# Samleo8/RadarSLAMPy

Measured on AMD Instinct MI355X. Metric: radar scan-pairs/sec (400x3768 polar), higher is better.
Workload: dtype u8/f32/f64

## Files before the change

### radarslampy_amd/csrc/engine.hip

```cpp
#include "roam_internal.h"
#include "retrack.h"
#include "kabsch_body.inc"
#include <algorithm>
#include <new>

#define KS ROAM_MAX_FEATURES
#define CART_CENTER 1012.0
#define M_PER_PX 0.0864
#define N_RETRACK 60
#define ROT_THR 0.2
#define TRANS_THR_SQ 4.0
#define ERR_THR 10.0f
#define TWO_PI 6.283185307179586476925286766559

#define RES_RING 8
enum { ST_PEAKS = 0, ST_WARP, ST_PYR, ST_KLT, ST_GRAPH, ST_CLIQUE, ST_KABSCH, ST_LM, ST_GLUE, ST_RETRACK, ST_COUNT };
static const char *kStageNames[ST_COUNT] = {"ingest_peaks", "warp_quantise", "pyramid", "klt", "consistency_graph",
                                            "max_clique", "kabsch", "mds_lm", "glue", "retrack"};

struct Engine {
    roam_engine_cfg cfg;
    int B = 0, W = 0, stage_cap = 0;
    PyrDesc pd;
    size_t rec_bytes = 0;
// ... 532 lines not shown
    if (e->scan_host) hipHostFree(e->scan_host);
    if (e->prior_host) hipHostFree(e->prior_host);
    if (e->results_host) hipHostFree(e->results_host);
    for (auto &ev : e->ev_res) if (ev) hipEventDestroy(ev);
    if (e->st_comm) { hipStreamSynchronize(e->st_comm); hipStreamDestroy(e->st_comm); }
    for (auto &ev : e->ev_kfx) if (ev) hipEventDestroy(ev);
    if (e->ev_pool) hipEventDestroy(e->ev_pool);
    for (auto &ev : e->ev_up_ring) if (ev) hipEventDestroy(ev);
    hipStreamSynchronize(ctx->stream2);
    hipStreamSynchronize(ctx->stream4);
    delete e;
    ctx->engine = nullptr;
    return ROAM_OK;
}

static int32_t fused_tables(roam_ctx *ctx, Engine *e)
{
    RtArgs &r = e->rt;
    if (r.fd_mapT) return ROAM_OK;
    const size_t npx = (size_t)e->W * e->W, R = (size_t)r.slots;
    uint32_t *mapT = nullptr, *boxtab = nullptr, *darktab = nullptr;
    bool ok = dalloc(ctx, e, &mapT, npx) && dalloc(ctx, e, &boxtab, retrack_fused_boxtab_words(e->W)) && dalloc(ctx, e, &darktab, retrack_darktab_words(e->W));
    ok = ok && dalloc(ctx, e, &r.fd_halo, R * 2 * (size_t)r.fd_halo_words) && dalloc(ctx, e, &r.fd_cc, R * 2048);
    if (!ok) return ROAM_E_HIP;
    HIP_TRY(ctx, launch_retrack_fused_tables(ctx->stream, e->warp_map, e->W, e->cfg.clip, mapT, boxtab, darktab));
    HIP_TRY(ctx, hipStreamSynchronize(ctx->stream));
    r.fd_boxtab = boxtab; r.fd_darktab = darktab;
    r.fd_mapT = mapT;
    return ROAM_OK;
}

int32_t roam_engine_create(roam_ctx *ctx, const roam_engine_cfg *cfg)
{
    if (!ctx) return ROAM_E_ARG;
    HIP_TRY(ctx, hipSetDevice(ctx->device));
    ARG_CHECK(ctx, cfg && cfg->lanes >= 1 && cfg->rows >= 1 && cfg->rows <= 1020 && cfg->clip >= 32 && cfg->clip <= 4094 && (cfg->clip / 2) % 2 == 0 &&
                       (int64_t)cfg->rows * cfg->stride < (1ll << 30) &&
                       cfg->payload_off >= 0 && cfg->stride >= cfg->payload_off + cfg->clip && cfg->pool_scans >= 1 &&
                       cfg->peaks_cap >= 1);
    roam_engine_destroy(ctx);
    Engine *e = new (std::nothrow) Engine();
    if (!e) return ROAM_E_HIP;
    ctx->engine = e;
    e->cfg = *cfg;
    if (!(e->cfg.keyframe_trans_m > 0.0)) e->cfg.keyframe_trans_m = 2.0;
    if (!(e->cfg.keyframe_rot_rad > 0.0)) e->cfg.keyframe_rot_rad = ROT_THR;
    const int B = e->B = cfg->lanes;
    e->lane_k.assign(B, 0);
    e->last_scan.assign(B, -1);
    e->prev_scan.assign(B, -1);
    e->lane_seen.assign(B, 0);
    e->slot_writes.assign((size_t)cfg->pool_scans, 0);
    e->W = 2 * (cfg->clip / 2);
    e->stage_cap = (cfg->clip + 1) / 2;
    pyr_desc_init(&e->pd, e->W, e->W);
    e->rec_bytes = (size_t)cfg->rows * cfg->stride;
    const int nw = KS / 64;
    bool ok = true;
    ok = ok && dalloc(ctx, e, &e->pool, e->rec_bytes * cfg->pool_scans + 64);
    ok = ok && dalloc(ctx, e, &e->pyr[0], (size_t)e->pd.lane_stride * B);
    ok = ok && dalloc(ctx, e, &e->pyr[1], (size_t)e->pd.lane_stride * B);
    ok = ok && dalloc(ctx, e, &e->pyr[2], (size_t)e->pd.lane_stride * B);
    ok = ok && dalloc(ctx, e, &e->pyr[3], (size_t)e->pd.lane_stride * B);
    ok = ok && dalloc(ctx, e, &e->pyr_dark, pyr_dark_words(e->W));
    ok = ok && dalloc(ctx, e, &e->warp_map, (size_t)e->W * e->W);
    ok = ok && dalloc(ctx, e, &e->row_stage, (size_t)B * cfg->rows * e->stage_cap);
    ok = ok && dalloc(ctx, e, &e->row_count, (size_t)B * cfg->rows);
    for (int i = 0; i < 3; i++) {
        ok = ok && dalloc(ctx, e, &e->peaks_out[i], (size_t)B * cfg->peaks_cap * 2);
        ok = ok && dalloc(ctx, e, &e->peaks_n[i], (size_t)B);
        ok = ok && dalloc(ctx, e, &e->scan_idx[i], 2 * (size_t)B);
    }
    if (ok && hipHostMalloc(reinterpret_cast<void **>(&e->scan_host), sizeof(int32_t) * 6 * (size_t)B, hipHostMallocDefault) != hipSuccess) {
        ROAM_SET_ERR(ctx, "engine: hipHostMalloc failed"); ok = false;
    }
    e->prior_bytes = ((size_t)B * 25 + 15) & ~(size_t)15;
    if (ok && hipHostMalloc(reinterpret_cast<void **>(&e->prior_host), 4 * e->prior_bytes, hipHostMallocDefault) != hipSuccess) {
        ROAM_SET_ERR(ctx, "engine: hipHostMalloc failed"); ok = false;
    }
    ok = ok && dalloc(ctx, e, &e->prior_dev, 4 * e->prior_bytes);
    ok = ok && dalloc(ctx, e, &e->feat, (size_t)B * KS * 2);
    ok = ok && dalloc(ctx, e, &e->feat_n, (size_t)B);
    ok = ok && dalloc(ctx, e, &e->klt_next, (size_t)B * KS * 2);
    ok = ok && dalloc(ctx, e, &e->klt_err, (size_t)B * KS);
    ok = ok && dalloc(ctx, e, &e->klt_status, (size_t)B * KS);
    ok = ok && dalloc(ctx, e, &e->good_old, (size_t)B * KS * 2);
    ok = ok && dalloc(ctx, e, &e->good_new, (size_t)B * KS * 2);
    ok = ok && dalloc(ctx, e, &e->good_idx, (size_t)B * KS);
    ok = ok && dalloc(ctx, e, &e->good_n, (size_t)B);
    ok = ok && dalloc(ctx, e, &e->adj, (size_t)B * KS * nw);
    ok = ok && dalloc(ctx, e, &e->cq_stack, (size_t)B * (KS + 2) * 2 * nw);
    ok = ok && dalloc(ctx, e, &e->cq_order, (size_t)B);
    ok = ok && dalloc(ctx, e, &e->cq_mask, (size_t)B * KS);
    ok = ok && dalloc(ctx, e, &e->cq_n, (size_t)B);
    ok = ok && dalloc(ctx, e, &e->cq_flags, (size_t)B);
    ok = ok && dalloc(ctx, e, &e->kab_src, (size_t)B * KS * 2);
    ok = ok && dalloc(ctx, e, &e->kab_tgt, (size_t)B * KS * 2);
    ok = ok && dalloc(ctx, e, &e->kab_out, (size_t)B * 6);
    ok = ok && dalloc(ctx, e, &e->in_n, (size_t)B);
    ok = ok && dalloc(ctx, e, &e->kf_pose, (size_t)B * 3);
    ok = ok && dalloc(ctx, e, &e->kf_vel, (size_t)B * 3) && dalloc(ctx, e, &e->kf_scan, (size_t)B) && dalloc(ctx, e, &e->kf_fresh, (size_t)B) &&
         dalloc(ctx, e, &e->kf_live, (size_t)B) && dalloc(ctx, e, &e->map_n, (size_t)B);
    ok = ok && dalloc(ctx, e, &e->kf_und, (size_t)B * KS * 2);
    ok = ok && dalloc(ctx, e, &e->kf_und_tmp, (size_t)B * KS * 2);
    ok = ok && dalloc(ctx, e, &e->pose, (size_t)B * 3);
    ok = ok && dalloc(ctx, e, &e->vel, (size_t)B * 3);
    ok = ok && dalloc(ctx, e, &e->T_wj0, (size_t)B * 9);
    ok = ok && dalloc(ctx, e, &e->T_init, (size_t)B * 9);
    ok = ok && dalloc(ctx, e, &e->p_w, (size_t)B * KS * 2);
    ok = ok && dalloc(ctx, e, &e->p_jt, (size_t)B * KS * 2);
    ok = ok && dalloc(ctx, e, &e->lm_work, (size_t)B * ((size_t)(2 * KS + 3) * 9 + KS));
    ok = ok && dalloc(ctx, e, &e->lm_out, (size_t)B * 6);
    ok = ok && dalloc(ctx, e, &e->lm_nfev, (size_t)B);
    ok = ok && dalloc(ctx, e, &e->lm_big, (size_t)2 * (1 + B));
    ok = ok && dalloc(ctx, e, &e->lm_info, (size_t)B);
    ok = ok && dalloc(ctx, e, &e->results, (size_t)B * RES_RING);
    if (ok && hipHostMalloc(reinterpret_cast<void **>(&e->results_host), sizeof(roam_lane_result) * (size_t)B * RES_RING, hipHostMallocDefault) != hipSuccess) {
        ROAM_SET_ERR(ctx, "engine: hipHostMalloc failed"); ok = false;
    }
    { const char *se = getenv("ROAM_STAGE_EVENTS"); e->stage_ev = !(se && se[0] == '0'); e->stage_ev_forced = se && (se[0] == '0' || se[0] == '1'); }
    e->rt_on = cfg->retrack_on_device != 0;
    if (ok && e->rt_on) {
        RtArgs &r = e->rt;
        memset(&r, 0, sizeof(r));
        const double step = (10.0 - 0.01) / 2.0;
        r.sigma1 = 1.0 * step + 0.01; r.sigma2 = 10.0; r.threshold = 0.0005;
        r.size1 = (int)(3 * r.sigma1); r.size2 = (int)(3 * r.sigma2);
        r.W = e->W; r.rows = cfg->rows; r.cols = cfg->clip; r.stride = cfg->stride; r.payload_off = cfg->payload_off;
        r.rec_bytes = (int64_t)e->rec_bytes;
        const int R = r.slots = std::max(1, std::min(B, cfg->retrack_slots > 0 ? cfg->retrack_slots : 2048));
        const size_t npx = (size_t)e->W * e->W;
        if (e->W > 2048) { ROAM_SET_ERR(ctx, "engine: device retrack needs a Cartesian image of at most 2048 x 2048"); roam_engine_destroy(ctx); return ROAM_E_ARG; }
        ok = ok && dalloc(ctx, e, &r.rt_n, 2) && dalloc(ctx, e, &r.rt_lane, (size_t)B) && dalloc(ctx, e, &r.rt_scan, (size_t)B);
        r.SP = (e->W + 15) & ~15;
        ok = ok && dalloc(ctx, e, &r.S, (size_t)r.SP * e->W * R);
        ok = ok && dalloc(ctx, e, const_cast<uint32_t **>(&r.boxtab), retrack_boxtab_words(e->W));
        ok = ok && dalloc(ctx, e, const_cast<uint32_t **>(&r.darktab), retrack_darktab_words(e->W));
        ok = ok && dalloc(ctx, e, const_cast<uint32_t **>(&r.phlist), retrack_phase_words(e->W));
        ok = ok && dalloc(ctx, e, &r.colT, (size_t)std::min(R, RT_TWO_PASS_SLOTS) * ((e->W + 63) / 64) * e->W);
        ok = ok && dalloc(ctx, e, &r.col_done, (size_t)std::min(R, RT_TWO_PASS_SLOTS) * 64);
        {
            const char *fv = getenv("ROAM_FUSED_DETECT");
            r.fused = (fv && fv[0] == '1') ? 1 : 0;
            e->det_side.chunk = getenv("ROAM_DET_SIDE") ? atoi(getenv("ROAM_DET_SIDE")) : ((B >= 2048 && r.slots >= 2048) ? 1024 : 0);
            r.fd_halo_words = (int64_t)retrack_fused_halo_words(e->W);
        }
        const size_t D = (size_t)B;
        ok = ok && dalloc(ctx, e, &r.cand_rc, D * BP_MAX_PTS) && dalloc(ctx, e, &r.cand_val, D * BP_MAX_PTS) && dalloc(ctx, e, &r.cand_n, D);
        ok = ok && dalloc(ctx, e, &r.tasks, D * BP_MAX_TASKS) && dalloc(ctx, e, &r.pairs, D * (BP_MAX_PAIRS + 1));
        ok = ok && dalloc(ctx, e, &r.order, D * (BP_MAX_PAIRS + 1)) && dalloc(ctx, e, &r.ovbits, D * ((BP_MAX_PAIRS + 31) / 32 + 1));
        ok = ok && dalloc(ctx, e, &r.bigtab, D * 2 * 131072);
        ok = ok && dalloc(ctx, e, &r.kp, D * BP_MAX_PTS * 3) && dalloc(ctx, e, &r.kp_n, D) && dalloc(ctx, e, &r.slot_flags, D);
        ok = ok && dalloc(ctx, e, &r.ssc_work, D * 4 * BP_MAX_PTS) && dalloc(ctx, e, &r.sel, D * BP_MAX_PTS) && dalloc(ctx, e, &r.sel_n, D) && dalloc(ctx, e, &r.blob_order_buf, D);
    }
    if (!ok) { roam_engine_destroy(ctx); return ROAM_E_HIP; }
    if (e->rt_on) {
        if (hipError_t er = retrack_init(); er != hipSuccess) {
            ROAM_SET_ERR(ctx, "retrack_init failed: %s", hipGetErrorString(er));
            roam_engine_destroy(ctx);
            return ROAM_E_HIP;
        }
        RtArgs &r = e->rt;
        r.pool = e->pool; r.map = e->warp_map; r.feat = e->feat; r.feat_n = e->feat_n; r.vel = e->vel; r.kf_und = e->kf_und; r.res = nullptr;
    }
    for (auto &ev : e->ev_res)
        if (hipEventCreateWithFlags(&ev, hipEventDisableTiming) != hipSuccess) { ROAM_SET_ERR(ctx, "hipEventCreate failed"); roam_engine_destroy(ctx); return ROAM_E_HIP; }
    e->slot_seq.assign((size_t)cfg->pool_scans, 0);
    for (auto &ev : e->ev_up_ring)
        if (hipEventCreateWithFlags(&ev, hipEventDisableTiming) != hipSuccess) { ROAM_SET_ERR(ctx, "hipEventCreate failed"); roam_engine_destroy(ctx); return ROAM_E_HIP; }
    if (hipEventCreateWithFlags(&e->ev_pool, hipEventDisableTiming) != hipSuccess) {
        ROAM_SET_ERR(ctx, "hipEventCreate failed"); roam_engine_destroy(ctx); return ROAM_E_HIP;
    }
    for (auto &ev : e->ev) {
        if (hipEventCreate(&ev) != hipSuccess) { ROAM_SET_ERR(ctx, "hipEventCreate failed"); roam_engine_destroy(ctx); return ROAM_E_HIP; }
    }
    if (hipEventCreate(&e->ev_join) != hipSuccess ||
        hipEventCreate(&e->ev_pk0) != hipSuccess || hipEventCreate(&e->ev_pk1) != hipSuccess ||
        hipEventCreateWithFlags(&e->ev_warp, hipEventDisableTiming) != hipSuccess || hipEventCreateWithFlags(&e->ev_idx, hipEventDisableTiming) != hipSuccess ||
        hipEventCreateWithFlags(&e->ev_peaks, hipEventDisableTiming) != hipSuccess) {
        ROAM_SET_ERR(ctx, "hipEventCreate failed"); roam_engine_destroy(ctx); return ROAM_E_HIP;
    }
    for (int i = 0; i < 4; i++)
        if (hipEventCreateWithFlags(&e->ev_klt[i], hipEventDisableTiming) != hipSuccess || hipEventCreateWithFlags(&e->ev_g4[i], hipEventDisableTiming) != hipSuccess) {
            ROAM_SET_ERR(ctx, "hipEventCreate failed"); roam_engine_destroy(ctx); return ROAM_E_HIP;
        }
    e->ev_ok = true;
    e->tr_ok = true;
    HIP_TRY(ctx, launch_warp_map(ctx->stream, cfg->rows, cfg->clip, e->warp_map));
    HIP_TRY(ctx, launch_pyr_dark(ctx->stream, e->warp_map, e->W, e->W, cfg->clip, e->pyr_dark));
    if (e->rt_on) HIP_TRY(ctx, launch_retrack_boxtab(ctx->stream, e->warp_map, e->W, cfg->clip, const_cast<uint32_t *>(e->rt.boxtab)));
    if (e->rt_on) HIP_TRY(ctx, launch_retrack_darktab(ctx->stream, e->warp_map, e->W, cfg->clip, const_cast<uint32_t *>(e->rt.darktab)));
    if (e->rt_on && e->rt.fused) { const int32_t rc_ = fused_tables(ctx, e); if (rc_ != ROAM_OK) { roam_engine_destroy(ctx); return rc_; } }
    HIP_TRY(ctx, hipStreamSynchronize(ctx->stream));
    e->rt_image_px = (int64_t)e->W * e->W;
    if (e->rt_on && e->W <= 2048 && B >= RT_TWO_PASS_SLOTS) {
        e->rt_image_px = 0;
        const size_t npx = (size_t)e->W * e->W, ndt = retrack_darktab_words(e->W), nph = retrack_phase_words(e->W);
        uint32_t *stage = nullptr;
        HIP_TRY(ctx, hipHostMalloc(reinterpret_cast<void **>(&stage), (npx + ndt + nph) * 4, hipHostMallocDefault));
        uint32_t *mh = stage, *dh = stage + npx;
        std::vector<uint32_t> ph(nph, 0u);
        hipError_t ec = hipMemcpyAsync(mh, e->warp_map, npx * 4, hipMemcpyDeviceToHost, ctx->stream);
        if (ec == hipSuccess) ec = hipMemcpyAsync(dh, e->rt.darktab, ndt * 4, hipMemcpyDeviceToHost, ctx->stream);
        if (ec == hipSuccess) ec = hipStreamSynchronize(ctx->stream);
        bool okp = ec == hipSuccess && retrack_build_phases(mh, dh, e->W, cfg->clip, ph.data());
        if (okp) {
            memcpy(stage + npx + ndt, ph.data(), nph * 4);
            ec = hipMemcpyAsync(const_cast<uint32_t *>(e->rt.phlist), stage + npx + ndt, nph * 4, hipMemcpyHostToDevice, ctx->stream);
            if (ec == hipSuccess) ec = hipStreamSynchronize(ctx->stream);
        }
        (void)hipHostFree(stage);
        if (!okp || ec != hipSuccess) { ROAM_SET_ERR(ctx, "retrack: phase list (%s)", ec != hipSuccess ? hipGetErrorString(ec) : "image too large"); roam_engine_destroy(ctx); return ec != hipSuccess ? ROAM_E_HIP : ROAM_E_ARG; }
        for (uint32_t i = 0; i < ph[0]; i++) {
            const int br = retrack_band_rows(), band = (int)(ph[1 + i] & 255u), g = (int)((ph[1 + i] >> 8) & 15u), hrows = std::min(br, e->W - br * band);
            for (int w = 0; w < 4; w++)
                if ((ph[1 + i] >> (12 + w)) & 1u) e->rt_image_px += (int64_t)hrows * std::max(0, std::min(64, e->W - (g * 256 + 64 * w)));
        }
    }
    return ROAM_OK;
}

#define ENGINE()                                  \
    if (!ctx) return ROAM_E_ARG;                  \
    Engine *e = ctx->engine;                      \
    if (!e) { ROAM_SET_ERR(ctx, "engine not created"); return ROAM_E_STATE; } \
    HIP_TRY(ctx, hipSetDevice(ctx->device))

int32_t roam_engine_upload_scan(roam_ctx *ctx, int32_t pool_idx, const uint8_t *rec)
{
    ENGINE();
    ARG_CHECK(ctx, rec && pool_idx >= 0 && pool_idx < e->cfg.pool_scans);
    e->slot_writes[(size_t)pool_idx]++;
    HIP_TRY(ctx, hipMemcpyAsync(e->pool + (size_t)pool_idx * e->rec_bytes, rec, e->rec_bytes, hipMemcpyHostToDevice, ctx->stream));
    HIP_TRY(ctx, hipStreamSynchronize(ctx->stream));
    return ROAM_OK;
}

int32_t roam_engine_upload_scans_async(roam_ctx *ctx, int32_t pool_idx0, int32_t n, const uint8_t *host_records, int64_t host_stride)
{
    ENGINE();
    ARG_CHECK(ctx, host_records && n >= 1 && pool_idx0 >= 0 && pool_idx0 + n <= e->cfg.pool_scans && (host_stride == 0 || host_stride >= (int64_t)e->rec_bytes));
    hipPointerAttribute_t at;
    const hipError_t pa = hipPointerGetAttributes(&at, host_records);
    if (pa != hipSuccess || (at.type != hipMemoryTypeHost && at.type != hipMemoryTypeManaged && at.type != hipMemoryTypeDevice)) {
        (void)hipGetLastError();
        ROAM_SET_ERR(ctx, "upload_scans_async: host_records is not pinned host memory (hipHostMalloc / hipHostRegister / roam_host_alloc)");
        return ROAM_E_ARG;
    }
    const uint8_t *dev_alias = at.devicePointer ? static_cast<const uint8_t *>(at.devicePointer) : host_records;
    const int width = e->cfg.payload_off + e->cfg.clip;
    hipLaunchKernelGGL(ingest_rows_kernel, dim3((e->cfg.rows + 3) / 4, n), dim3(256), 0, ctx->stream3, dev_alias, host_stride,
                       e->pool + (size_t)pool_idx0 * e->rec_bytes, (int64_t)e->rec_bytes, e->cfg.rows, e->cfg.stride, width);
    HIP_TRY(ctx, hipGetLastError());
    HIP_TRY(ctx, hipEventRecord(ctx->ev_up, ctx->stream3));
    e->up_seq++;
    for (int i = 0; i < n; i++) { e->slot_seq[(size_t)pool_idx0 + i] = e->up_seq; e->slot_writes[(size_t)pool_idx0 + i]++; }
    HIP_TRY(ctx, hipEventRecord(e->ev_up_ring[e->up_seq & 15], ctx->stream3));
    e->uploads_pending = true;
    return ROAM_OK;
}

int32_t roam_engine_fence(roam_ctx *ctx)
{
    ENGINE();
    HIP_TRY(ctx, hipEventRecord(ctx->ev_fence, ctx->stream));
    HIP_TRY(ctx, hipStreamWaitEvent(ctx->stream3, ctx->ev_fence, 0));
    return ROAM_OK;
}

int32_t roam_engine_copy_scan(roam_ctx *ctx, int32_t dst_idx, int32_t src_idx)
{
    ENGINE();
    ARG_CHECK(ctx, dst_idx >= 0 && dst_idx < e->cfg.pool_scans && src_idx >= 0 && src_idx < e->cfg.pool_scans);
    if (dst_idx != src_idx)
    {
        HIP_TRY(ctx, hipMemcpyAsync(e->pool + (size_t)dst_idx * e->rec_bytes, e->pool + (size_t)src_idx * e->rec_bytes,
                                    e->rec_bytes, hipMemcpyDeviceToDevice, ctx->stream));
        HIP_TRY(ctx, hipEventRecord(e->ev_pool, ctx->stream));
        e->pool_dirty = true;
        e->ap_pool_dirty = true;
        e->slot_writes[(size_t)dst_idx]++;
    }
    return ROAM_OK;
}

static WarpSrc pool_warp_src(Engine *e, const int32_t *lane_index)
{
    WarpSrc s = {e->pool, (int64_t)e->rec_bytes, (int64_t)e->cfg.stride, e->cfg.payload_off, 1, lane_index};
    return s;
}

static int32_t set_features_impl(roam_ctx *ctx, Engine *e, int32_t lane, const float *pts, int32_t K, int32_t kf_scan)
{
    float *f = e->feat + (size_t)lane * KS * 2;
    if (e->map_cap > 0) {
        hipLaunchKernelGGL(map_freeze_kernel, dim3(1), dim3(256), 0, ctx->stream, e->map_store, e->map_n, e->map_cap, lane,
                           e->kf_pose, e->kf_vel, e->feat_n, e->kf_scan, e->kf_und, e->kf_live, e->kf_fresh);
        HIP_TRY(ctx, hipGetLastError());
    }
    e->lane_k[lane] = K;
    if (K > 0) HIP_TRY(ctx, hipMemcpyAsync(f, pts, sizeof(float) * 2 * (size_t)K, hipMemcpyHostToDevice, ctx->stream));
    HIP_TRY(ctx, hipMemcpyAsync(e->feat_n + lane, &K, sizeof(int32_t), hipMemcpyHostToDevice, ctx->stream));
    HIP_TRY(ctx, hipMemcpyAsync(e->kf_pose + 3 * (size_t)lane, e->pose + 3 * (size_t)lane, sizeof(double) * 3,
                                hipMemcpyDeviceToDevice, ctx->stream));
    HIP_TRY(ctx, hipMemcpyAsync(e->kf_vel + 3 * (size_t)lane, e->vel + 3 * (size_t)lane, sizeof(double) * 3,
                                hipMemcpyDeviceToDevice, ctx->stream));
// ... 976 lines not shown
```

### radarslampy_amd/csrc/retrack.h

```cpp
#pragma once
#include "roam_internal.h"
#include "blobprune.h"

#define RT_TWO_PASS_SLOTS 200
enum { RT_F_CAND_OVERFLOW = 1, RT_F_TREE_OVERFLOW = 2, RT_F_PAIR_OVERFLOW = 4, RT_F_FEAT_OVERFLOW = 8 };

struct RtArgs {
    int W, rows, cols, stride, payload_off, slots, size1, size2;
    int64_t rec_bytes;
    double sigma1, sigma2, threshold;
    const uint8_t *pool;
    const uint32_t *map;
    const uint32_t *phlist;
    const uint32_t *boxtab;
    const uint32_t *darktab;
    float *feat;
    int32_t *feat_n;
    const double *vel;
    double *kf_und;
    roam_lane_result *res;
    int32_t *rt_n, *rt_lane, *rt_scan;
    double *S;
    int32_t *col_done;
    double *colT;
    int SP;
    uint32_t *cand_rc;
    double *cand_val;
    int32_t *cand_n;
    BpTask *tasks;
    uint32_t *pairs;
    uint16_t *order;
    uint32_t *ovbits;
    uint16_t *bigtab;
    double *kp;
    int32_t *kp_n, *slot_flags;
    int32_t *ssc_work;
    int32_t *sel, *sel_n;
    int32_t *blob_order_buf;
    const int32_t *blob_order;
    int fused;
    const uint32_t *fd_mapT;
    const uint32_t *fd_boxtab;
    const uint32_t *fd_darktab;
    double *fd_halo;
    int64_t fd_halo_words;
    double *fd_cc;
};

hipError_t launch_retrack_collect(hipStream_t st, const roam_lane_result *res, const int32_t *scan_idx, int B, int force_all, const RtArgs &a);
#define RT_TRACE_CHUNKS 16
struct RtSide { hipStream_t st; hipEvent_t ev_i[4], ev_d[4]; int chunk; };
bool retrack_sided(const RtArgs &a, int B, const RtSide *side);
hipError_t launch_retrack(hipStream_t st, const RtArgs &a, int B, hipEvent_t *trace = nullptr, int ntrace = 0, hipEvent_t after_order = nullptr, const RtSide *side = nullptr);
hipError_t launch_ssc_batch(hipStream_t st, const double *kp, int64_t kp_stride, const int32_t *count, int kp_cap, int P,
                            int num_ret, double tol, int cols, int rows, int32_t *work, int32_t *sel, int32_t *n_sel,
                            const int32_t *n_active, int first);
hipError_t launch_retrack_part(hipStream_t st, const RtArgs &a, int P, int which);
hipError_t launch_retrack_emit(hipStream_t st, const RtArgs &a, int P);
hipError_t retrack_init();
size_t retrack_boxtab_words(int W);
size_t retrack_phase_words(int W);
int retrack_band_rows();
bool retrack_build_phases(const uint32_t *map_host, const uint32_t *darktab_host, int W, int cols, uint32_t *out);
hipError_t launch_retrack_boxtab(hipStream_t st, const uint32_t *map, int W, int cols, uint32_t *boxtab);
size_t retrack_darktab_words(int W);
size_t retrack_fused_boxtab_words(int W);
size_t retrack_fused_halo_words(int W);
hipError_t launch_retrack_fused_tables(hipStream_t st, const uint32_t *map, int W, int cols, uint32_t *mapT, uint32_t *boxtab, uint32_t *darktab);
hipError_t launch_retrack_darktab(hipStream_t st, const uint32_t *map, int W, int cols, uint32_t *darktab);
```

### radarslampy_amd/csrc/retrack_blobs.hip

```cpp
#include "retrack_geom.h"
#include "npsort_wave.h"
#include "ssc_body.inc"

__global__ __launch_bounds__(256) void rt_emit_kernel(RtArgs a, int first)
{
    __shared__ uint32_t key[BP_MAX_PTS];
    __shared__ double val[BP_MAX_PTS];
    const int ls = blockIdx.x, slot = first + ls;
    if (slot >= *a.rt_n) return;
    const int t = threadIdx.x;
    const int n = min(a.cand_n[ls], BP_MAX_PTS);
    uint32_t *crc = a.cand_rc + (int64_t)ls * BP_MAX_PTS;
    double *cval = a.cand_val + (int64_t)ls * BP_MAX_PTS;
    for (int i = t; i < n; i += 256) { key[i] = crc[i]; val[i] = cval[i]; }
    __syncthreads();
    for (int i = t; i < n; i += 256) {
        const uint32_t k = key[i];
        int rank = 0;
        for (int j = 0; j < n; j++) rank += key[j] < k ? 1 : 0;
        crc[rank] = k;
        cval[rank] = val[i];
    }
}

// ... 86 lines not shown
        }
    __syncthreads();
}


__device__ int rb_build_node_wave(BpPt *pt, int start, int end, BpNode &nd, int lane, uint16_t *Lp, uint16_t *Rp)
{
    nd.start = (int16_t)start; nd.end = (int16_t)end; nd.less = nd.greater = -1; nd.split_dim = -1; nd.split = 0;
    if (end - start <= BP_LEAF) return -1;
    int mx0 = -32768, mn0 = 32767, mx1 = -32768, mn1 = 32767;
    for (int j = start + lane; j < end; j += 64) {
        const int v0 = rb_key(pt, j, 0), v1 = rb_key(pt, j, 1);
        mx0 = max(mx0, v0); mn0 = min(mn0, v0); mx1 = max(mx1, v1); mn1 = min(mn1, v1);
    }
    for (int m = 32; m >= 1; m >>= 1) {
        mx0 = max(mx0, __shfl_xor(mx0, m)); mn0 = min(mn0, __shfl_xor(mn0, m));
        mx1 = max(mx1, __shfl_xor(mx1, m)); mn1 = min(mn1, __shfl_xor(mn1, m));
    }
    int d = 0, size = 0;
    if (mx0 - mn0 > size) { d = 0; size = mx0 - mn0; }
    if (mx1 - mn1 > size) { d = 1; size = mx1 - mn1; }
    if (size <= 0) return -1;
    const int half = (end - start) / 2;
    rb_nth_element_wave(pt, start, start + half, end, d, lane, Lp, Rp);
    int split = rb_key(pt, start + half, d);
    const uint64_t below = (1ull << lane) - 1ull;
    int nL = 0, nR = 0;
    for (int c0 = start; c0 < end; c0 += 64) {
        const int pos = c0 + lane;
        const int k = pos < end ? rb_key(pt, pos, d) : 0;
        const bool ge = pos < end && k >= split, lt = pos < end && k < split;
        const uint64_t bl = __ballot(ge), br = __ballot(lt);
        if (ge) Lp[nL + __popcll(bl & below)] = (uint16_t)pos;
        if (lt) Rp[nR + __popcll(br & below)] = (uint16_t)pos;
        nL += __popcll(bl); nR += __popcll(br);
    }
    __syncthreads();
    {
        const int nm = min(nL, nR);
        int kk = 0;
        for (int i0 = 0; i0 < nm; i0 += 64) {
            const int i = i0 + lane;
            const uint64_t bal = __ballot(i < nm && Lp[i] < Rp[nR - 1 - i]);
            kk += __popcll(bal);
            if (__popcll(bal) < min(64, nm - i0)) break;
        }
        for (int i = lane; i < kk; i += 64) { const int x = Lp[i], y = Rp[nR - 1 - i]; const BpPt t = pt[x]; pt[x] = pt[y]; pt[y] = t; }
    }
    __syncthreads();
    int p = start + nR;
    if (p == start || p == end) {
        if (lane == 0) {
            if (p == start) {
                int j = start; split = rb_key(pt, j, d);
                for (int k = start + 1; k < end; k++) if (rb_key(pt, k, d) < split) { j = k; split = rb_key(pt, j, d); }
                const BpPt t = pt[start]; pt[start] = pt[j]; pt[j] = t;
            } else {
                int j = end - 1; split = rb_key(pt, j, d);
                for (int k = start; k < end - 1; k++) if (rb_key(pt, k, d) > split) { j = k; split = rb_key(pt, j, d); }
                const BpPt t = pt[end - 1]; pt[end - 1] = pt[j]; pt[j] = t;
            }
        }
        __syncthreads();
        split = rb_key(pt, p == start ? start : end - 1, d);
        p = p == start ? start + 1 : end - 1;
    }
    nd.split_dim = (int16_t)d; nd.split = split;
    return p;
}

template <bool TLDS, typename ORD>
__device__ int rb_pyset_order_wave(const uint32_t *pairs, int np, uint16_t *tabA, int capA, uint16_t *tabB, int capB, ORD *order, int lane)
{
    uint16_t *tab = tabA, *other = tabB;
    int cap_other = capB, cap_cur = capA;
    uint32_t mask = 7;
    if (lane < 8) tab[lane] = 0;
    __syncthreads();
    const uint64_t below = (1ull << lane) - 1ull;
    int fill = 0;
    auto insert_chunk = [&](uint16_t *t, uint32_t msk, const ORD *src, int p0, int cnt) {
        const int key1 = lane < cnt ? (src ? (int)src[p0 + lane] : p0 + lane + 1) : 0;
        const uint64_t h = key1 ? bp_tuple_hash(pairs[key1 - 1]) : 0ull;
        for (int j = 0; j < cnt; j++) {
            const uint64_t hj = ((uint64_t)(uint32_t)__builtin_amdgcn_readlane((int)(h >> 32), j) << 32) | (uint32_t)__builtin_amdgcn_readlane((int)(h & 0xffffffffull), j);
            const int kj = __builtin_amdgcn_readlane(key1, j);
            uint64_t perturb = hj;
            uint32_t i = (uint32_t)hj & msk;
            for (;;) {
                const int probes = (i + 9 <= msk) ? 9 : 0;
                int e = -1;
                for (int q = 0; q <= probes; q++) if (t[i + q] == 0) { e = (int)i + q; break; }
                if (e >= 0) { if (lane == 0) t[e] = (uint16_t)kj; break; }
                perturb >>= 5;
                i = (uint32_t)(((uint64_t)i * 5 + 1 + perturb) & msk);
            }
            if (!TLDS) __builtin_amdgcn_fence(__ATOMIC_SEQ_CST, "workgroup");
        }
    };
    for (int p = 0; p < np;) {
        int room = (int)(((uint64_t)mask * 3 + 4) / 5) - fill;
        if (room < 1) room = 1;
        const int cnt = min(min(64, np - p), room);
        insert_chunk(tab, mask, (const ORD *)nullptr, p, cnt);
        p += cnt; fill += cnt;
        __syncthreads();
        if ((uint64_t)fill * 5 >= (uint64_t)mask * 3) {
            const int minused = fill > 50000 ? fill * 2 : fill * 4;
            uint32_t newsize = 8;
            while ((int)newsize <= minused) newsize <<= 1;
            if ((int)newsize > cap_other) return -1;
            for (uint32_t k = lane; k < newsize; k += 64) other[k] = 0;
            int m = 0;
            for (uint32_t k0 = 0; k0 <= mask; k0 += 64) {
                const uint32_t k = k0 + lane;
                const int key = k <= mask ? (int)tab[k] : 0;
                const uint64_t bal = __ballot(key != 0);
                if (key) order[m + __popcll(bal & below)] = (ORD)key;
                m += __popcll(bal);
            }
            __syncthreads();
            for (int q = 0; q < m; q += 64) insert_chunk(other, newsize - 1, order, q, min(64, m - q));
            __syncthreads();
            uint16_t *t = tab; tab = other; other = t;
            const int c = cap_cur; cap_cur = cap_other; cap_other = c;
            mask = newsize - 1;
        }
    }
    __syncthreads();
    int m = 0;
    for (uint32_t k0 = 0; k0 <= mask; k0 += 64) {
        const uint32_t k = k0 + lane;
        const int key = k <= mask ? (int)tab[k] : 0;
        const uint64_t bal = __ballot(key != 0);
        if (key) order[m + __popcll(bal & below)] = (ORD)(key - 1);
        m += __popcll(bal);
    }
    __syncthreads();
    return m;
}

#ifdef RB_EXP_PROF
__device__ unsigned long long rb_prof[16];
extern "C" int roam_debug_blob_prof(unsigned long long *out, int reset)
{
    if (hipMemcpyFromSymbol(out, HIP_SYMBOL(rb_prof), sizeof(rb_prof)) != hipSuccess) return -1;
    if (reset) { unsigned long long z[16] = {0}; if (hipMemcpyToSymbol(HIP_SYMBOL(rb_prof), z, sizeof(z)) != hipSuccess) return -1; }
    return 0;
}
#define RB_P(k) { const unsigned long long tn_ = __builtin_readcyclecounter(); if (threadIdx.x == 0) rbp_[k] += tn_ - rbt_; rbt_ = tn_; }
#else
#define RB_P(k)
#endif
template <bool SMALL>
__device__ int rt_blobs_body(const RtArgs &a, int first, RtBlobLds<SMALL> &L, bool forced)
{
#ifdef RB_EXP_PROF
    unsigned long long rbp_[12] = {0}, rbt_ = __builtin_readcyclecounter();
#endif
    typedef RtBlobCap<SMALL> CP;
    const int ls = a.blob_order ? a.blob_order[blockIdx.x] : (int)blockIdx.x, slot = first + ls;
    if (slot >= *a.rt_n) return 0;
    const int lane = threadIdx.x;
    const int ncand = a.cand_n[ls];
    if (!SMALL && !forced && a.kp_n[ls] != RT_BLOBS_REDO) return 0;
    if (SMALL && ncand > CP::NP) {
        if (lane == 0) a.kp_n[ls] = RT_BLOBS_REDO;
        return 1;
    }
    const int n = min(ncand, BP_MAX_PTS);
    const uint32_t *crc = a.cand_rc + (int64_t)ls * BP_MAX_PTS;
    const double *cval = a.cand_val + (int64_t)ls * BP_MAX_PTS;
    double *kp = a.kp + (int64_t)ls * BP_MAX_PTS * 3;
    int flags = ncand > BP_MAX_PTS ? RT_F_CAND_OVERFLOW : 0;
    double *sval = reinterpret_cast<double *>(L.tabB);
    for (int i = lane; i < n; i += 64) sval[i] = cval[i];
    __syncthreads();
    for (int i0 = lane; i0 < n; i0 += 256) {
        double vi[4];
        int rank[4] = {0, 0, 0, 0};
#pragma unroll
        for (int u = 0; u < 4; u++) vi[u] = i0 + 64 * u < n ? sval[i0 + 64 * u] : 0.0;
        for (int j = 0; j < n; j++) {
            const double vj = sval[j];
#pragma unroll
            for (int u = 0; u < 4; u++) rank[u] += (vj > vi[u] || (vj == vi[u] && j < i0 + 64 * u)) ? 1 : 0;
        }
#pragma unroll
        for (int u = 0; u < 4; u++) {
            const int i = i0 + 64 * u;
            if (i < n) {
                const uint32_t p = crc[i];
                L.xy[2 * rank[u]] = (int16_t)(p >> 16); L.xy[2 * rank[u] + 1] = (int16_t)((p >> 2) & 0x3fff); L.lay[rank[u]] = (uint8_t)(p & 3);
            }
        }
    }
    __syncthreads();
    RB_P(0)
    BpPt *pt = reinterpret_cast<BpPt *>(L.tabB);
    for (int i = lane; i < n; i += 64)
        pt[i].v = (uint64_t)(uint16_t)L.xy[2 * i] | ((uint64_t)(uint16_t)L.xy[2 * i + 1] << 16) | ((uint64_t)i << 32);
    int nn = 0;
    if (n > 0) {
        {
            int mn0 = 32767, mx0 = -32768, mn1 = 32767, mx1 = -32768;
            for (int i = lane; i < n; i += 64) {
                const int v0 = L.xy[2 * i], v1 = L.xy[2 * i + 1];
                mn0 = min(mn0, v0); mx0 = max(mx0, v0); mn1 = min(mn1, v1); mx1 = max(mx1, v1);
            }
            for (int d = 32; d >= 1; d >>= 1) {
                mn0 = min(mn0, __shfl_xor(mn0, d)); mx0 = max(mx0, __shfl_xor(mx0, d));
                mn1 = min(mn1, __shfl_xor(mn1, d)); mx1 = max(mx1, __shfl_xor(mx1, d));
            }
            if (lane == 0) { L.nbox[0][0] = (int16_t)mn0; L.nbox[0][1] = (int16_t)mx0; L.nbox[0][2] = (int16_t)mn1; L.nbox[0][3] = (int16_t)mx1; }
        }
        if (lane == 0) { L.nodes[0].start = 0; L.nodes[0].end = (int16_t)n; }
        nn = 1;
        __syncthreads();
        for (int lo = 0, hi = 1; lo < hi && nn > 0;) {
            for (int base = lo; base < hi; base += 64) {
                const int me = base + lane;
                const bool act = me < hi;
                BpNode nd;
                int p = -1, start = 0, end = 0;
                if (act) { start = L.nodes[me].start; end = L.nodes[me].end; }
                uint64_t big = __ballot(act && end - start > RB_WAVE_MIN);
                const uint64_t bigs = big;
                while (big) {
                    const int j = __ffsll((long long)big) - 1;
                    big &= big - 1;
                    BpNode ndw;
                    const int pw = rb_build_node_wave(pt, __builtin_amdgcn_readlane(start, j), __builtin_amdgcn_readlane(end, j), ndw, lane,
                                                      reinterpret_cast<uint16_t *>(L.pl), reinterpret_cast<uint16_t *>(L.pl) + CP::NP);
                    if (lane == j) { p = pw; nd = ndw; }
                }
                if (act && !((bigs >> lane) & 1ull)) p = bp_build_node(L.xy, pt, start, end, nd);
                const uint64_t bal = __ballot(act && p >= 0);
                const int kids = 2 * __popcll(bal);
                if (nn + kids > CP::NNODE) { nn = -1; break; }
                if (act) {
                    if (p >= 0) {
                        const int c0 = nn + 2 * __popcll(bal & ((1ull << lane) - 1ull));
                        nd.less = (int16_t)c0; nd.greater = (int16_t)(c0 + 1);
                        L.nodes[c0].start = (int16_t)start; L.nodes[c0].end = (int16_t)p;
                        L.nodes[c0 + 1].start = (int16_t)p; L.nodes[c0 + 1].end = (int16_t)end;
                        for (int k = 0; k < 4; k++) L.nbox[c0][k] = L.nbox[c0 + 1][k] = L.nbox[me][k];
                        L.nbox[c0][2 * nd.split_dim + 1] = (int16_t)nd.split;
                        L.nbox[c0 + 1][2 * nd.split_dim] = (int16_t)nd.split;
                    }
                    L.nodes[me] = nd;
                }
                nn += kids;
            }
            if (nn < 0) break;
            __syncthreads();
            lo = hi; hi = nn;
        }
    }
    __syncthreads();
    if (SMALL && nn < 0) {
        if (lane == 0) a.kp_n[ls] = RT_BLOBS_REDO;
        return 1;
    }
    for (int i = lane; i < n; i += 64) L.idx[i] = (int16_t)(pt[i].v >> 32);
    __syncthreads();
    RB_P(1)
    BpTask *tasks = a.tasks + (int64_t)ls * BP_MAX_TASKS;
    int nt = 0;
    double ub = 0;
    {
        bool any2l = false;
        for (int i = lane; i < n; i += 64) any2l = any2l || L.lay[i] == 2;
        const bool any2 = __ballot(any2l) != 0;
        const double r = 2 * (any2 ? a.sigma2 : a.sigma1) * 1.4142135623730951;
        ub = r * r;
    }
    if (nn < 0) flags |= RT_F_TREE_OVERFLOW;
    else if (n > 1) {
        const int t_gt = (int)floor(ub), t_lt = (int)ceil(ub);
        uint32_t *fa = a.pairs + (int64_t)ls * (BP_MAX_PAIRS + 1), *fb = fa + BP_MAX_TASKS;
        if (lane == 0) fa[0] = 0u;
        int F = 1;
        bool over = false;
        const uint64_t below = (1ull << lane) - 1ull;
        for (;;) {
            __syncthreads();
            int total = 0;
            bool open = false;
            for (int c0 = 0; c0 < F; c0 += 64) {
                const bool act = c0 + lane < F;
                const uint32_t it = act ? fa[c0 + lane] : 0u;
                const int na = it & 1023, nb = (it >> 10) & 1023;
                int m = act ? (int)(it >> 20) : 2;
                uint32_t ch[4];
                int cnt = 0;
                if (act && m >= 2) { ch[0] = it; cnt = 1; }
                else if (act) {
                    const BpNode n1 = L.nodes[na], n2 = L.nodes[nb];
                    const bool l1 = n1.split_dim == -1, l2 = n2.split_dim == -1;
                    bool pruned = false;
                    if (m == 0) {
                        int mind = 0, maxd = 0;
                        for (int k = 0; k < 2; k++) {
                            const int a0 = L.nbox[na][2 * k], a1 = L.nbox[na][2 * k + 1], b0 = L.nbox[nb][2 * k], b1 = L.nbox[nb][2 * k + 1];
                            const int lo = max(max(a0 - b1, b0 - a1), 0), hi = max(a1 - b0, b1 - a0);
                            mind += lo * lo; maxd += hi * hi;
                        }
                        if (mind > t_gt) pruned = true;
                        else if (maxd < t_lt) m = 1;
                    }
                    const uint32_t mm = (uint32_t)m << 20;
                    if (pruned) cnt = 0;
                    else if (l1 && l2) { ch[0] = (uint32_t)na | ((uint32_t)nb << 10) | ((m == 0 ? 2u : 3u) << 20); cnt = 1; }
                    else if (m == 1) {
                        if (l1) { ch[0] = na | ((uint32_t)n2.less << 10) | mm; ch[1] = na | ((uint32_t)n2.greater << 10) | mm; cnt = 2; }
                        else if (na == nb) {
                            ch[0] = n1.less | ((uint32_t)n2.less << 10) | mm; ch[1] = n1.less | ((uint32_t)n2.greater << 10) | mm;
                            ch[2] = n1.greater | ((uint32_t)n2.greater << 10) | mm; cnt = 3;
                        } else { ch[0] = n1.less | ((uint32_t)nb << 10) | mm; ch[1] = n1.greater | ((uint32_t)nb << 10) | mm; cnt = 2; }
                    } else {
                        if (l1) { ch[0] = na | ((uint32_t)n2.less << 10); ch[1] = na | ((uint32_t)n2.greater << 10); cnt = 2; }
                        else if (l2) { ch[0] = n1.less | ((uint32_t)nb << 10); ch[1] = n1.greater | ((uint32_t)nb << 10); cnt = 2; }
                        else {
                            ch[0] = n1.less | ((uint32_t)n2.less << 10); ch[1] = n1.less | ((uint32_t)n2.greater << 10); cnt = 2;
                            if (na != nb) ch[cnt++] = n1.greater | ((uint32_t)n2.less << 10);
                            ch[cnt++] = n1.greater | ((uint32_t)n2.greater << 10);
                        }
                    }
                }
                const uint64_t b1 = __ballot(cnt >= 1), b2 = __ballot(cnt >= 2), b3 = __ballot(cnt >= 3), b4 = __ballot(cnt >= 4);
                const int off = total + __popcll(b1 & below) + __popcll(b2 & below) + __popcll(b3 & below) + __popcll(b4 & below);
                const int sum = __popcll(b1) + __popcll(b2) + __popcll(b3) + __popcll(b4);
                if (total + sum > BP_MAX_TASKS) { over = true; break; }
                for (int j = 0; j < cnt; j++) fb[off + j] = ch[j];
                open = open || (cnt > 0 && (ch[0] >> 20) < 2u);
                total += sum;
            }
            if (over) break;
            uint32_t *t = fa; fa = fb; fb = t;
            F = total;
            if (!__ballot(open)) break;
        }
        __syncthreads();
        if (over) flags |= RT_F_TREE_OVERFLOW;
        else {
            nt = F;
            for (int i = lane; i < nt; i += 64) {
                const uint32_t it = fa[i];
                tasks[i].a = (int16_t)(it & 1023); tasks[i].b = (int16_t)((it >> 10) & 1023); tasks[i].mode = (int32_t)(it >> 20) - 2;
            }
        }
    }
    __syncthreads();
    RB_P(2)
    uint32_t *pairs = a.pairs + (int64_t)ls * (BP_MAX_PAIRS + 1);
    int np = 0;
    for (int t = 0; t < nt; t++) {
        const BpTask tk = tasks[t];
        const BpNode n1 = L.nodes[tk.a], n2 = L.nodes[tk.b];
        const int la = n1.end - n1.start, lb = n2.end - n2.start, tot = la * lb;
        const bool same = tk.a == tk.b;
        for (int base = 0; base < tot; base += 64) {
            const int k = base + lane;
            bool ok = k < tot;
            int pi = 0, pj = 0;
            if (ok) {
                const int i = n1.start + k / lb, j = n2.start + k % lb;
                if (same && j <= i) ok = false;
                else {
                    pi = L.idx[i]; pj = L.idx[j];
                    if (!tk.mode) {
                        const double d0 = (double)L.xy[2 * pi] - (double)L.xy[2 * pj], d1 = (double)L.xy[2 * pi + 1] - (double)L.xy[2 * pj + 1];
                        ok = d0 * d0 + d1 * d1 <= ub;
                    }
                }
            }
            const uint64_t bal = __ballot(ok);
            const int o = np + __popcll(bal & ((1ull << lane) - 1ull));
            if (ok && o < BP_MAX_PAIRS) { pairs[o] = bp_pack(pi, pj); if (o < CP::NPL) L.pl[o] = bp_pack(pi, pj); }
            np += __popcll(bal);
        }
    }
    if (np > BP_MAX_PAIRS) { flags |= RT_F_PAIR_OVERFLOW; np = BP_MAX_PAIRS; }
    __syncthreads();
    RB_P(3)
    if (SMALL && np > CP::LDS_PAIRS) {
        if (lane == 0) a.kp_n[ls] = RT_BLOBS_REDO;
        return 1;
    }
    const bool lds_set = np <= CP::LDS_PAIRS, lds_pl = np <= CP::NPL;
    uint32_t *ovb = lds_set ? L.ovbits : a.ovbits + (int64_t)ls * ((BP_MAX_PAIRS + 31) / 32 + 1);
    for (int w0 = 0; w0 < np; w0 += 64) {
        const int k = w0 + lane;
        bool ov = false;
        if (k < np) {
            const uint32_t pr = lds_pl ? L.pl[k] : pairs[k];
            const int i = (int)(pr >> 16), j = (int)(pr & 0xffffu);
            ov = bp_overlaps((double)L.xy[2 * i], (double)L.xy[2 * i + 1], L.lay[i] == 2 ? a.sigma2 : a.sigma1,
                             (double)L.xy[2 * j], (double)L.xy[2 * j + 1], L.lay[j] == 2 ? a.sigma2 : a.sigma1, 0.5);
        }
        const uint64_t bal = __ballot(ov);
        if (lane == 0) { ovb[w0 >> 5] = (uint32_t)bal; ovb[(w0 >> 5) + 1] = (uint32_t)(bal >> 32); }
    }
    __syncthreads();
    RB_P(4)
    uint16_t *order = a.order + (int64_t)ls * (BP_MAX_PAIRS + 1);
    {
        int m;
        if (lds_pl) m = rb_pyset_order_wave<true>(L.pl, np, L.tabA, CP::CAPA, L.tabB, CP::CAPB, order, lane);
        else if (lds_set) m = rb_pyset_order_wave<true>(pairs, np, L.tabA, CP::CAPA, L.tabB, CP::CAPB, order, lane);
        else {
            uint16_t *big = a.bigtab + (int64_t)ls * 2 * 131072;
            m = rb_pyset_order_wave<false>(pairs, np, big, 131072, big + 131072, 131072, order, lane);
        }
        if (m != np) flags |= RT_F_PAIR_OVERFLOW;
        if (lane == 0) L.vals[2] = m < 0 ? 0 : m;
    }
    __syncthreads();
    RB_P(5)
    const int m = L.vals[2];
    uint32_t *cl = reinterpret_cast<uint32_t *>(L.tabB);
    int ncl = 0;
    for (int k0 = 0; k0 < m; k0 += 64) {
        const int k = k0 + lane;
        bool ov = false;
        uint32_t pr = 0;
        if (k < m) {
            const int q = order[k];
            ov = (ovb[q >> 5] >> (q & 31)) & 1u;
            if (ov) pr = lds_pl ? L.pl[q] : pairs[q];
        }
        const uint64_t bal = __ballot(ov);
        const int o = ncl + __popcll(bal & ((1ull << lane) - 1ull));
        if (ov && o < CP::NCL) cl[o] = pr;
        ncl += __popcll(bal);
    }
    __syncthreads();
    if (lane == 0) {
        if (ncl <= CP::NCL) {
            for (int k = 0; k < ncl; k++) {
                const uint32_t pr = cl[k];
                const int i = (int)(pr >> 16), j = (int)(pr & 0xffffu);
                if (L.lay[i] == 0 || L.lay[j] == 0) continue;
                if (L.lay[i] > L.lay[j]) L.lay[j] = 0; else L.lay[i] = 0;
            }
        } else {
            for (int k = 0; k < m; k++) {
                const int q = order[k];
                if (!((ovb[q >> 5] >> (q & 31)) & 1u)) continue;
                const uint32_t pr = pairs[q];
                const int i = (int)(pr >> 16), j = (int)(pr & 0xffffu);
                if (L.lay[i] == 0 || L.lay[j] == 0) continue;
                if (L.lay[i] > L.lay[j]) L.lay[j] = 0; else L.lay[i] = 0;
            }
        }
        L.vals[1] = flags;
    }
    __syncthreads();
    RB_P(6)
    int mb = 0;
    for (int i0 = 0; i0 < n; i0 += 64) {
        const int i = i0 + lane;
        const int ly = i < n ? (int)L.lay[i] : 0;
        const int16_t x = i < n ? L.xy[2 * i] : (int16_t)0, y = i < n ? L.xy[2 * i + 1] : (int16_t)0;
        const uint64_t bal = __ballot(ly != 0);
        __syncthreads();
        if (ly) { const int o = mb + __popcll(bal & ((1ull << lane) - 1ull)); L.xy[2 * o] = x; L.xy[2 * o + 1] = y; L.lay[o] = (uint8_t)ly; }
        mb += __popcll(bal);
        __syncthreads();
    }
    RB_P(7)
    rb_aquicksort_wave(L.lay, mb, L.idx, lane, L.st, reinterpret_cast<uint16_t *>(L.pl), reinterpret_cast<uint16_t *>(L.pl) + CP::NP);
    RB_P(8)
    for (int q = lane; q < mb; q += 64) {
        const int i = L.idx[q];
        kp[3 * q] = (double)L.xy[2 * i]; kp[3 * q + 1] = (double)L.xy[2 * i + 1]; kp[3 * q + 2] = L.lay[i] == 2 ? a.sigma2 : a.sigma1;
    }
    if (lane == 0) { a.kp_n[ls] = mb; a.slot_flags[ls] = L.vals[1]; }
    RB_P(9)
#ifdef RB_EXP_PROF
    if (lane == 0) for (int k = 0; k < 12; k++) atomicAdd(&rb_prof[k], rbp_[k]);
    if (lane == 0) { atomicAdd(&rb_prof[12], 1ull); atomicAdd(&rb_prof[13], (unsigned long long)n); atomicAdd(&rb_prof[14], (unsigned long long)mb); }
#endif
    return 0;
}

template <bool SMALL>
__global__ __launch_bounds__(64) void rt_blobs_kernel(RtArgs a, int first)
{
    __shared__ RtBlobLds<SMALL> L;
    rt_blobs_body<SMALL>(a, first, L, false);
}
__global__ __launch_bounds__(64) void rt_book_kernel(RtArgs a, int first)
{
    __shared__ union U_ {
        RtBlobLds<true> s; RtBlobLds<false> f;
        struct { uint32_t key[BP_MAX_PTS]; double val[BP_MAX_PTS]; } e;
        uint32_t bitmap[SSC_BATCH_BITMAP_BYTES / 4];
        __device__ U_() {}
    } L;
    const int ls = blockIdx.x, slot = first + ls, lane = threadIdx.x;
    if (slot >= *a.rt_n) return;
    {
        const int n = min(a.cand_n[ls], BP_MAX_PTS);
        uint32_t *crc = a.cand_rc + (int64_t)ls * BP_MAX_PTS;
        double *cval = a.cand_val + (int64_t)ls * BP_MAX_PTS;
        for (int i = lane; i < n; i += 64) { L.e.key[i] = crc[i]; L.e.val[i] = cval[i]; }
        __syncthreads();
        for (int i0 = lane; i0 < n; i0 += 256) {
            uint32_t k[4];
            int rank[4] = {0, 0, 0, 0};
#pragma unroll
            for (int u = 0; u < 4; u++) k[u] = i0 + 64 * u < n ? L.e.key[i0 + 64 * u] : 0u;
            for (int j = 0; j < n; j++) {
                const uint32_t kj = L.e.key[j];
#pragma unroll
                for (int u = 0; u < 4; u++) rank[u] += kj < k[u] ? 1 : 0;
            }
#pragma unroll
            for (int u = 0; u < 4; u++)
                if (i0 + 64 * u < n) { crc[rank[u]] = k[u]; cval[rank[u]] = L.e.val[i0 + 64 * u]; }
        }
        __builtin_amdgcn_fence(__ATOMIC_SEQ_CST, "agent");
        __syncthreads();
    }
    if (rt_blobs_body<true>(a, first, L.s, false)) {
        __syncthreads();
        rt_blobs_body<false>(a, first, L.f, true);
    }
    __builtin_amdgcn_fence(__ATOMIC_SEQ_CST, "agent");
    __syncthreads();
    const int nk = min(a.kp_n[ls], BP_MAX_PTS);
    if (nk <= 0) { if (lane == 0) a.sel_n[ls] = 0; return; }
    ssc_body(a.kp + (int64_t)ls * BP_MAX_PTS * 3, nk, 200, 0.1, a.W, a.W, a.ssc_work + (int64_t)ls * 4 * BP_MAX_PTS,
             a.sel + (int64_t)ls * BP_MAX_PTS, a.sel_n + ls, L.bitmap, SSC_BATCH_BITMAP_BYTES);
}

hipError_t launch_retrack_emit(hipStream_t st, const RtArgs &a, int P)
{
    hipLaunchKernelGGL(rt_emit_kernel, dim3(P), dim3(256), 0, st, a, 0);
    return hipGetLastError();
}

hipError_t launch_retrack_bookkeeping(hipStream_t st, const RtArgs &a, int B, hipEvent_t after_order)
{
    RtArgs ab = a;
    ab.blob_order = nullptr;
    if (B < 256) {
        hipLaunchKernelGGL(rt_book_kernel, dim3(B), dim3(64), 0, st, ab, 0);
        return hipGetLastError();
    }
    hipLaunchKernelGGL(rt_emit_kernel, dim3(B), dim3(256), 0, st, a, 0);
    if (B >= 512 && a.blob_order_buf) {
        if (hipError_t e = launch_order_by_count(st, a.cand_n, B, BP_MAX_PTS, a.blob_order_buf, 1); e != hipSuccess) return e;
        ab.blob_order = a.blob_order_buf;
    }
    if (hipError_t e = after_order ? hipEventRecord(after_order, st) : hipSuccess; e != hipSuccess) return e;
    hipLaunchKernelGGL(rt_blobs_kernel<true>, dim3(B), dim3(64), 0, st, ab, 0);
    hipLaunchKernelGGL(rt_blobs_kernel<false>, dim3(B), dim3(64), 0, st, ab, 0);
    return launch_ssc_batch(st, a.kp, (int64_t)BP_MAX_PTS * 3, a.kp_n, BP_MAX_PTS, B, 200, 0.1, a.W, a.W, a.ssc_work, a.sel, a.sel_n, a.rt_n, 0);
}
```

Before: 55390.

## Compact redo slots into a worklist for the full-size blob kernel

The small-capacity blob pass now appends the slots it cannot handle to a device worklist through an atomic counter. The full-capacity pass runs a persistent grid of about twice the CU count that walks only that list, instead of launching one block per slot that mostly exits early. The last block to finish resets the counters for the next call. This cuts empty-block launch and scheduling overhead in exchange for atomics and a grid-stride loop, which could leave CUs idle when many slots need redoing.

```diff
diff --git a/radarslampy_amd/csrc/engine.hip b/radarslampy_amd/csrc/engine.hip
--- a/radarslampy_amd/csrc/engine.hip
+++ b/radarslampy_amd/csrc/engine.hip
@@ -708,6 +708,8 @@
         ok = ok && dalloc(ctx, e, &r.bigtab, D * 2 * 131072);
         ok = ok && dalloc(ctx, e, &r.kp, D * BP_MAX_PTS * 3) && dalloc(ctx, e, &r.kp_n, D) && dalloc(ctx, e, &r.slot_flags, D);
         ok = ok && dalloc(ctx, e, &r.ssc_work, D * 4 * BP_MAX_PTS) && dalloc(ctx, e, &r.sel, D * BP_MAX_PTS) && dalloc(ctx, e, &r.sel_n, D) && dalloc(ctx, e, &r.blob_order_buf, D);
+        ok = ok && dalloc(ctx, e, &r.redo_list, D) && dalloc(ctx, e, &r.redo_n, 2);
+        r.cu_count = ctx->cu_count;
     }
     if (!ok) { roam_engine_destroy(ctx); return ROAM_E_HIP; }
     if (e->rt_on) {
diff --git a/radarslampy_amd/csrc/retrack.h b/radarslampy_amd/csrc/retrack.h
--- a/radarslampy_amd/csrc/retrack.h
+++ b/radarslampy_amd/csrc/retrack.h
@@ -34,6 +34,8 @@
     uint16_t *bigtab;
     double *kp;
     int32_t *kp_n, *slot_flags;
+    int32_t *redo_list, *redo_n;
+    int cu_count;
     int32_t *ssc_work;
     int32_t *sel, *sel_n;
     int32_t *blob_order_buf;
diff --git a/radarslampy_amd/csrc/retrack_blobs.hip b/radarslampy_amd/csrc/retrack_blobs.hip
--- a/radarslampy_amd/csrc/retrack_blobs.hip
+++ b/radarslampy_amd/csrc/retrack_blobs.hip
@@ -262,20 +262,22 @@
 #else
 #define RB_P(k)
 #endif
+__device__ __forceinline__ void rt_blobs_redo(const RtArgs &a, int ls)
+{
+    a.kp_n[ls] = RT_BLOBS_REDO;
+    if (a.redo_list) a.redo_list[atomicAdd(a.redo_n, 1)] = ls;
+}
 template <bool SMALL>
-__device__ int rt_blobs_body(const RtArgs &a, int first, RtBlobLds<SMALL> &L, bool forced)
+__device__ int rt_blobs_body(const RtArgs &a, int ls, RtBlobLds<SMALL> &L)
 {
 #ifdef RB_EXP_PROF
     unsigned long long rbp_[12] = {0}, rbt_ = __builtin_readcyclecounter();
 #endif
     typedef RtBlobCap<SMALL> CP;
-    const int ls = a.blob_order ? a.blob_order[blockIdx.x] : (int)blockIdx.x, slot = first + ls;
-    if (slot >= *a.rt_n) return 0;
     const int lane = threadIdx.x;
     const int ncand = a.cand_n[ls];
-    if (!SMALL && !forced && a.kp_n[ls] != RT_BLOBS_REDO) return 0;
     if (SMALL && ncand > CP::NP) {
-        if (lane == 0) a.kp_n[ls] = RT_BLOBS_REDO;
+        if (lane == 0) rt_blobs_redo(a, ls);
         return 1;
     }
     const int n = min(ncand, BP_MAX_PTS);
@@ -369,7 +371,7 @@
     }
     __syncthreads();
     if (SMALL && nn < 0) {
-        if (lane == 0) a.kp_n[ls] = RT_BLOBS_REDO;
+        if (lane == 0) rt_blobs_redo(a, ls);
         return 1;
     }
     for (int i = lane; i < n; i += 64) L.idx[i] = (int16_t)(pt[i].v >> 32);
@@ -495,7 +497,7 @@
     __syncthreads();
     RB_P(3)
     if (SMALL && np > CP::LDS_PAIRS) {
-        if (lane == 0) a.kp_n[ls] = RT_BLOBS_REDO;
+        if (lane == 0) rt_blobs_redo(a, ls);
         return 1;
     }
     const bool lds_set = np <= CP::LDS_PAIRS, lds_pl = np <= CP::NPL;
@@ -599,7 +601,17 @@
 __global__ __launch_bounds__(64) void rt_blobs_kernel(RtArgs a, int first)
 {
     __shared__ RtBlobLds<SMALL> L;
-    rt_blobs_body<SMALL>(a, first, L, false);
+    if (SMALL) {
+        const int ls = a.blob_order ? a.blob_order[blockIdx.x] : (int)blockIdx.x;
+        if (first + ls < *a.rt_n) rt_blobs_body<SMALL>(a, ls, L);
+        return;
+    }
+    const int n = *a.redo_n;
+    for (int i = blockIdx.x; i < n; i += gridDim.x) {
+        rt_blobs_body<SMALL>(a, a.redo_list[i], L);
+        __syncthreads();
+    }
+    if (threadIdx.x == 0 && atomicAdd(a.redo_n + 1, 1) == (int)gridDim.x - 1) { a.redo_n[0] = 0; a.redo_n[1] = 0; }
 }
 __global__ __launch_bounds__(64) void rt_book_kernel(RtArgs a, int first)
 {
@@ -634,9 +646,9 @@
         __builtin_amdgcn_fence(__ATOMIC_SEQ_CST, "agent");
         __syncthreads();
     }
-    if (rt_blobs_body<true>(a, first, L.s, false)) {
-        __syncthreads();
-        rt_blobs_body<false>(a, first, L.f, true);
+    if (rt_blobs_body<true>(a, ls, L.s)) {
+        __syncthreads();
+        rt_blobs_body<false>(a, ls, L.f);
     }
     __builtin_amdgcn_fence(__ATOMIC_SEQ_CST, "agent");
     __syncthreads();
@@ -657,6 +669,7 @@
     RtArgs ab = a;
     ab.blob_order = nullptr;
     if (B < 256) {
+        ab.redo_list = nullptr;
         hipLaunchKernelGGL(rt_book_kernel, dim3(B), dim3(64), 0, st, ab, 0);
         return hipGetLastError();
     }
@@ -667,6 +680,6 @@
     }
     if (hipError_t e = after_order ? hipEventRecord(after_order, st) : hipSuccess; e != hipSuccess) return e;
     hipLaunchKernelGGL(rt_blobs_kernel<true>, dim3(B), dim3(64), 0, st, ab, 0);
-    hipLaunchKernelGGL(rt_blobs_kernel<false>, dim3(B), dim3(64), 0, st, ab, 0);
+    hipLaunchKernelGGL(rt_blobs_kernel<false>, dim3(std::min(B, 2 * std::max(1, a.cu_count))), dim3(64), 0, st, ab, 0);
     return launch_ssc_batch(st, a.kp, (int64_t)BP_MAX_PTS * 3, a.kp_n, BP_MAX_PTS, B, 200, 0.1, a.W, a.W, a.ssc_work, a.sel, a.sel_n, a.rt_n, 0);
 }
```

Result: slower. 54600 (-1.4%).
